# stm233/image-compression-for-machine

Hardware: AMD Instinct MI355X
Metric: images/sec (256x256) cnn-hyperprior (WACNN) training step (higher is better)
Workload: dtype f32; 1 GPU; cnn (WACNN N=192 M=320) train step, lambda=0.0067 MSE, batch 16/GPU synthetic 256x256, Adam lr 1e-4 + aux Adam, clip 1.0; global_batch=16, parallelism=dp1

## Files before the change

image-compression-for-machine_amd/csrc/conv_1x1.hip:

```cpp
#include <cstdlib>
#include "conv_common.h"

namespace icm {

template <int TCO, int TPX>
__global__ __launch_bounds__(256, 2) void conv1x1_kernel(const ConvDesc d) {
  constexpr int DB = 4;
  const int lane = threadIdx.x & 63;
  const int wave = __builtin_amdgcn_readfirstlane((int)(threadIdx.x >> 6));
  const ConvPtrs P = d.g[blockIdx.y];
  int bid = xcd_block_id();
  const int cb = bid % d.ncb, ptile = bid / d.ncb;
  const int h = lane >> 5, l31 = lane & 31;
  const int HW = d.pg.H * d.pg.W;
  const int NP = d.pg.N * HW;
  const int p_base = (ptile * 4 + wave) * (32 * TPX);
  if (p_base >= NP) return;
  unsigned voff[TPX];
  int pn[TPX], phw[TPX];
  bool pv[TPX];
#pragma unroll
  for (int tp = 0; tp < TPX; ++tp) {
    const int p = p_base + tp * 32 + l31;
    pv[tp] = p < NP;
// ... 44 lines not shown
      const int q = q0 + u;
      if (q >= nq) break;
      float bv[4][TPX];
#pragma unroll
      for (int j = 0; j < 4; ++j)
#pragma unroll
        for (int tp = 0; tp < TPX; ++tp) bv[j][tp] = bq[u][j][tp];
      if (act == ICM_ACT_GELU) {
#pragma unroll
        for (int j = 0; j < 4; ++j)
#pragma unroll
          for (int tp = 0; tp < TPX; ++tp) bv[j][tp] = gelu_f(bv[j][tp]);
      } else if (act == ICM_ACT_SQUARE) {
#pragma unroll
        for (int j = 0; j < 4; ++j)
#pragma unroll
          for (int tp = 0; tp < TPX; ++tp) bv[j][tp] *= bv[j][tp];
      }
      loadB(bq[u], q + DB);
      const char* sp = wbase + (long long)min(q + 2, nq - 1) * qstride;
#pragma unroll
      for (int a = 0; a < TCO; ++a) {
#pragma unroll
        for (int tp = 0; tp < TPX; ++tp)
#pragma unroll
          for (int j = 0; j < 4; ++j)
            acc[a][tp] = __builtin_amdgcn_mfma_f32_32x32x2f32(aq[u & 1][a][j], bv[j][tp], acc[a][tp], 0, 0, 0);
        aq[u & 1][a] = *reinterpret_cast<const f32x4*>(sp + wl[a]);
        __builtin_amdgcn_sched_barrier(0);
      }
    }
  }

  int zero[TPX];
#pragma unroll
  for (int tp = 0; tp < TPX; ++tp) zero[tp] = 0;
  epilogue_dispatch<TCO, TPX, !(TCO == 3 && TPX == 2)>(d, P, acc, cot0, h, pn, zero, phw, pv);
}

struct Cfg1x1 {
  int tco, tpx;
  void (*fn)(const ConvDesc);
  float eff;
};
static const Cfg1x1 kCfgs1x1[] = {
    {6, 1, conv1x1_kernel<6, 1>, 1.0f},  {5, 1, conv1x1_kernel<5, 1>, 1.0f}, {4, 1, conv1x1_kernel<4, 1>, 0.97f},
    {3, 2, conv1x1_kernel<3, 2>, 1.0f},  {2, 2, conv1x1_kernel<2, 2>, 0.7f}, {1, 2, conv1x1_kernel<1, 2>, 0.6f},
    {3, 1, conv1x1_kernel<3, 1>, 0.95f}, {2, 1, conv1x1_kernel<2, 1>, 0.6f},
};

int plan_conv1x1(const icm_conv_args& a, int ngroups, int g_force_1x1, ConvPlan& p) {
  if (g_force_1x1 == 0) return -1;
  if (a.KH != 1 || a.KW != 1 || a.stride != 1 || a.pad != 0 || a.pixel_shuffle || (a.Cin % 8) != 0) return -1;
  if (a.OH != a.H || a.OW != a.W) return -1;
  const int ncot = cdiv(a.Cout, 32);
  const long long NP = (long long)a.N * a.H * a.W;
  int best = -1, best_pad = 1 << 30;
  const int ncfg = (int)(sizeof(kCfgs1x1) / sizeof(kCfgs1x1[0]));
  for (int i = 0; i < ncfg; ++i) best_pad = std::min(best_pad, cdiv(ncot, kCfgs1x1[i].tco) * kCfgs1x1[i].tco);
  float best_score = -1.0f;
  for (int i = 0; i < ncfg; ++i) {
    const Cfg1x1& k = kCfgs1x1[i];
    if (cdiv(ncot, k.tco) * k.tco != best_pad) continue;
    const long long waves = ((NP + 32 * k.tpx - 1) / (32 * k.tpx)) * cdiv(ncot, k.tco) * ngroups;
    const float score = (float)std::min<long long>(waves, 2048) * k.eff;
    if (score > best_score) {
      best_score = score;
      best = i;
    }
  }
  {
    static const int force = env_int("ICM_1X1_CFG", -1);
    if (force >= 0 && force < ncfg) best = force;
  }
  const Cfg1x1& c = kCfgs1x1[best];
  const int ncb = cdiv(ncot, c.tco);
  const long long strips = (NP + 32 * c.tpx - 1) / (32 * c.tpx);
  static const long long kMinWaves = env_ll("ICM_1X1_MIN_WAVES", 1024);
  static const int kShortK = env_int("ICM_1X1_SHORT_K", 384);
  const long long need = a.Cin <= kShortK ? kMinWaves / 2 : kMinWaves;
  if (g_force_1x1 < 0 && strips * ncb * ngroups < need) return -1;
  const long long nblk = ((strips + 3) / 4) * ncb;
  if (nblk <= 0 || nblk > 0x7fffffffLL) return ICM_ERR_ARG;
  p = ConvPlan{};
  p.family = kFam1x1; p.row = best; p.g.ckm = 1; p.ncb = ncb; p.nblk = nblk; p.block = 256;
  return ICM_OK;
}

int launch_conv1x1(ConvDesc& d, const icm_conv_args& a, const ConvPlan& p, int ngroups, hipStream_t stream) {
  d.pg.H = a.H; d.pg.W = a.W; d.pg.N = a.N; d.pg.C = a.Cin; d.pg.act = a.pro_act; d.pg.bs = a.x_bs;
  d.OHf = a.H; d.OWf = a.W; d.OHv = a.H; d.OWv = a.W;
  d.out_sy = d.out_sx = 1;
  d.ntaps = 1;
  d.tiles_x = d.tiles_y = d.tiles_n = 1;
  d.nchunks8 = a.Cin / 8; d.ckm = p.g.ckm;
  hipLaunchKernelGGL(kCfgs1x1[p.row].fn, dim3((unsigned)p.nblk, ngroups, 1), dim3(p.block), 0, stream, d);
  ICM_CHECK_LAUNCH();
  return ICM_OK;
}

}
```

image-compression-for-machine_amd/csrc/conv_common.h:

```cpp
#pragma once
#include <type_traits>
#include "icm_common.h"

namespace icm {

#define ICM_MAX_TAPS 32
#define ICM_MAX_GROUPS 12

struct ConvPtrs {
  const float* x;
  const float* wp;
  const float* bias;
  float* y;
  const float* res;
  const float* aux;
  const float* aux2;
  float* y2;
};

struct ConvDesc {
  ConvPtrs g[ICM_MAX_GROUPS];
  long long y_bs, res_bs, aux_bs, aux2_bs, y2_bs;
  PatchGeom pg;
  int Cout, OHf, OWf;
  int OHv, OWv;
  int out_sy, out_oy, out_sx, out_ox;
  int iy0, ix0;
  int ntaps;
  int lgTW, lgTH, lgTI;
  int tiles_x, tiles_y, tiles_n;
  int ncot, nchunks8, ckm, ncb;
  int epi, accum, ps2;
  int tapoff[ICM_MAX_TAPS];
};

inline void fill_conv_ptrs(ConvPtrs (&g)[ICM_MAX_GROUPS], const icm_conv_args* arr, int ngroups, long long wp_off) {
  for (int gi = 0; gi < ICM_MAX_GROUPS; ++gi) {
    const icm_conv_args& s = arr[gi < ngroups ? gi : 0];
    g[gi] = ConvPtrs{s.x, s.wp + wp_off, s.bias, s.y, s.res, s.aux, s.aux2, s.y2};
  }
}
inline void fill_conv_desc(ConvDesc& d, const icm_conv_args* arr, int ngroups, long long wp_off) {
  const icm_conv_args& a = arr[0];
  fill_conv_ptrs(d.g, arr, ngroups, wp_off);
  d.y_bs = a.y_bs; d.res_bs = a.res_bs; d.aux_bs = a.aux_bs; d.aux2_bs = a.aux2_bs; d.y2_bs = a.y2_bs;
  d.Cout = a.Cout; d.ncot = (a.Cout + 31) / 32;
  d.epi = a.epi; d.accum = a.accum;
}

enum ConvFamily { kFamStaged = 0, kFamKs8 = 1, kFam1x1 = 2, kFamWino44 = 3, kFamWino8 = 4 };
struct Geometry {
  int lgTW, lgTH, lgTI, PH, PW, PWh, PWrow, PP, CS, tiles_x, tiles_y, tiles_n, ckm;
  size_t lds_bytes;
};
struct ConvPlan {
  int family;
  int row;
  Geometry g;
  int ncb;
  long long nblk;
  int block, vec4, dma;
};
struct WinoGeom {
  int lgTX, lgTY, lgTI, tiles_x, tiles_y, tiles_n, nchunks8, nsteps;
};
struct WinoPlan {
  WinoGeom g;
  int tco, w8, px_fast, ncb;
  long long nblk;
  size_t lds_bytes;
};

constexpr bool epi_reads_res(int e) { return e == ICM_EPI_RES || e == ICM_EPI_RES_GELU || e == ICM_EPI_RES_MUL_DGELU; }
constexpr bool epi_reads_aux(int e) {
  return e == ICM_EPI_GDN || e == ICM_EPI_IGDN || e == ICM_EPI_MUL_DGELU || e == ICM_EPI_AXPY2 || e == ICM_EPI_LRP ||
         e == ICM_EPI_RES_MUL_DGELU;
}
constexpr bool epi_reads_aux2(int e) { return e == ICM_EPI_AXPY2; }
constexpr bool epi_writes_side(int e) { return e == ICM_EPI_GDN || e == ICM_EPI_IGDN || e == ICM_EPI_LRP; }
constexpr bool epi_may_gelu(int e) { return e == ICM_EPI_NONE || e == ICM_EPI_RES || e == ICM_EPI_RES_GELU; }

template <int EPI>
__device__ __forceinline__ float epi_apply(float v, float rv, float av, float& side) {
  if constexpr (EPI == ICM_EPI_RES) v += rv;
  if constexpr (EPI == ICM_EPI_RES_GELU) v += gelu_f(rv);
  if constexpr (EPI == ICM_EPI_GDN || EPI == ICM_EPI_IGDN) {
    side = v;
    v = av * (EPI == ICM_EPI_GDN ? rsqrtf(v) : sqrtf(v));
  }
  if constexpr (EPI == ICM_EPI_MUL_DGELU) v *= dgelu_f(av);
  if constexpr (EPI == ICM_EPI_RES_MUL_DGELU) v = (v + rv) * dgelu_f(av);
  if constexpr (EPI == ICM_EPI_AXPY2) v = rv + 2.0f * av * v;
  if constexpr (EPI == ICM_EPI_LRP) {
    side = tanhf(v);
    v = av + 0.5f * side;
  }
  return v;
}
template <class Off>
__device__ __forceinline__ void epi_materialise(float& v, const float* y, float* y2, Off off, bool ok) {
  const float gv = gelu_f(v);
  if (y2 == y) v = gv;
  else if (ok) y2[off] = gv;
}

template <int... Kinds>
struct EpiKinds {
  static constexpr bool has(int epi) { return ((epi == Kinds) || ...); }
  template <class F>
  static __device__ __forceinline__ void dispatch(int epi, F&& f) {
    static_assert(((Kinds == ICM_EPI_NONE) || ...), "ICM_EPI_NONE is the fallback of every kernel");
    const bool hit = ((Kinds != ICM_EPI_NONE && epi == Kinds ? (f(std::integral_constant<int, Kinds>{}), true) : false) || ...);
    if (!hit) f(std::integral_constant<int, ICM_EPI_NONE>{});
  }
};
using EpiAll = EpiKinds<ICM_EPI_NONE, ICM_EPI_RES, ICM_EPI_RES_GELU, ICM_EPI_GDN, ICM_EPI_IGDN, ICM_EPI_MUL_DGELU,
                        ICM_EPI_AXPY2, ICM_EPI_LRP, ICM_EPI_RES_MUL_DGELU>;
using EpiKs8 = EpiKinds<ICM_EPI_NONE, ICM_EPI_RES, ICM_EPI_RES_GELU, ICM_EPI_MUL_DGELU, ICM_EPI_LRP, ICM_EPI_RES_MUL_DGELU>;
using EpiWino = EpiKinds<ICM_EPI_NONE, ICM_EPI_RES, ICM_EPI_RES_GELU, ICM_EPI_MUL_DGELU, ICM_EPI_RES_MUL_DGELU, ICM_EPI_LRP>;

template <int EPI, int half>
__device__ __forceinline__ void store_half_e(const ConvDesc& d, const ConvPtrs& P, const f32x16 acc, int cot, int h,
                                             int n, int oy, int ox, bool pvalid) {
  const int plane = d.OHf * d.OWf;
  constexpr bool kRes = epi_reads_res(EPI), kAux = epi_reads_aux(EPI), kAux2 = epi_reads_aux2(EPI);
  float* yb = P.y + n * d.y_bs;
  const float* resb = kRes ? P.res + n * d.res_bs : nullptr;
  const float* auxb = kAux ? P.aux + n * d.aux_bs : nullptr;
  const float* aux2b = kAux2 ? P.aux2 + n * d.aux2_bs : nullptr;
  float* y2b = P.y2 ? P.y2 + n * d.y2_bs : nullptr;
  const bool has_bias = P.bias != nullptr;
  {
    int off[8];
    bool ok[8];
    float bv[8], rv[8], av[8];
#pragma unroll
// ... 120 lines not shown
      }
    return;
  }
  constexpr int S = TPX * TCO * 2;
  EpiRegs R[2];
  epi_load<EPI>(d, P, cot0, 0, h, pn[0], poy[0], pox[0], pv[0], R[0]);
#pragma unroll
  for (int i = 0; i < S; ++i) {
    const int half = i & 1, a = (i >> 1) % TCO, tp = (i >> 1) / TCO;
    if (i + 1 < S) {
      const int i2 = i + 1;
      const int half2 = i2 & 1, a2 = (i2 >> 1) % TCO, tp2 = (i2 >> 1) / TCO;
      epi_load<EPI>(d, P, cot0 + a2, half2, h, pn[tp2], poy[tp2], pox[tp2], pv[tp2], R[i2 & 1]);
    }
    __builtin_amdgcn_sched_barrier(0);
    float a8[8];
#pragma unroll
    for (int q = 0; q < 8; ++q) a8[q] = acc[a][tp][half * 8 + q];
    epi_finish<EPI>(d, P, a8, R[i & 1]);
    __builtin_amdgcn_sched_barrier(0);
  }
}

template <int TCO, int TPX, bool PIPE2 = false>
__device__ __forceinline__ void epilogue_dispatch(const ConvDesc& d, const ConvPtrs& P, const f32x16 (&acc)[TCO][TPX],
                                                  int cot0, int h, const int (&pn)[TPX], const int (&poy)[TPX],
                                                  const int (&pox)[TPX], const bool (&pv)[TPX]) {
  EpiAll::dispatch(d.epi, [&](auto kind) {
    constexpr int EPI = decltype(kind)::value;
    epilogue_tiles<EPI, TCO, TPX, EPI == ICM_EPI_AXPY2 && PIPE2>(d, P, acc, cot0, h, pn, poy, pox, pv);
  });
}

int launch_conv_ks8(const ConvDesc& d, int tco, long long nblk, int ngroups, size_t lds_bytes, hipStream_t stream);

bool wino_supported(const icm_conv_args& a);
int plan_conv_wino(const icm_conv_args& a, int ngroups, WinoPlan& p);
int run_conv_wino(const icm_conv_args* arr, int ngroups, hipStream_t stream);
long long wino_transform_floats(const icm_conv_args& a);
int run_wino_transform(const icm_conv_args* arr, int ngroups, hipStream_t stream);

int plan_conv1x1(const icm_conv_args& a, int ngroups, int force_mode, ConvPlan& p);
int launch_conv1x1(ConvDesc& d, const icm_conv_args& a, const ConvPlan& p, int ngroups, hipStream_t stream);

}
```

image-compression-for-machine_amd/csrc/conv_igemm.hip:

```cpp
#include <climits>
#include <cstdlib>
#include <vector>
#include "conv_common.h"

namespace icm {

template <int WCO, int WPX, int TCO, int TPX, int KS = 1>
__global__ __launch_bounds__(512, (TCO * TPX <= 3) ? 4 : 2) void conv_igemm_kernel(const ConvDesc d) {
  extern __shared__ __attribute__((aligned(16))) float smem[];
  static_assert(WCO * WPX * KS == 4, "4 MFMA waves per workgroup");
  constexpr int BCO_T = WCO * TCO;
  constexpr int TS = (TCO * TPX == 1) ? 3 : ((TCO * TPX == 2) ? 2 : 1);
  const int tid = threadIdx.x, lane = tid & 63, wave = tid >> 6;
  const bool loader = wave >= 4;
  const ConvPtrs P = d.g[blockIdx.y];
  const PatchGeom& pg = d.pg;

  int bid = xcd_block_id();
  const int cb = bid % d.ncb;
  int pt = bid / d.ncb;
  const int tx_i = pt % d.tiles_x;
  pt /= d.tiles_x;
  const int ty_i = pt % d.tiles_y;
  const int tn_i = pt / d.tiles_y;
// ... 464 lines not shown
    }
    if (cost < best_cost) {
      best_cost = cost;
      best = i;
      bg = g;
    }
  }
  if (best1 >= 0 && best1_cost <= 1.2 * best_cost) {
    best = best1;
    bg = bg1;
  }
  return best;
}

static int plan_ks8(const icm_conv_args& a, int ngroups, const ConvClass& cls, const ClassShape& s, int S_in, Geometry& g) {
  static const int ks8_on = env_int("ICM_CONV_KS8", 1);
  static const long long ks8_max = env_ll("ICM_CONV_KS8_MAXWG", 256);
  static const long long ks8_min = env_ll("ICM_CONV_KS8_MINWG", 160);
  if (!(ks8_forced() || (ks8_on && !cfg_forced())) || S_in != 1 || s.ntaps <= 1 || a.pro_act != ICM_ACT_NONE ||
      !EpiKs8::has(a.epi) || a.x_seg_len != 0)
    return 0;
  const int tco = g_force_cfg == ICM_CONV_CFG_KS8_32X128 ? 1 : (g_force_cfg == ICM_CONV_CFG_KS8_64X64 ? 2 : (s.ncot >= 2 ? 2 : 1));
  g = make_geometry(tco == 2 ? 64 : 128, s.OHv, s.OWv, a.N, S_in, cls.ey, cls.ex, s.nchunks8, s.ntaps, 4);
  int ckm = std::max(1, std::min(s.nchunks8, 64 / s.ntaps));
  while (ckm > 1 && (size_t)2 * ckm * 8 * g.CS * sizeof(float) > 96 * 1024) --ckm;
  g.ckm = ckm;
  g.lds_bytes = std::max((size_t)2 * ckm * 8 * g.CS * sizeof(float), (size_t)8 * 4 * 16 * 64 * sizeof(float));
  const long long blocks = cdiv(s.ncot, tco) * tile_count(g) * ngroups;
  const bool fits = g.lds_bytes <= 160 * 1024 && fits_plane_map(g) && linear_patch(g);
  return (fits && (ks8_forced() || (blocks <= ks8_max && blocks >= ks8_min && tco == 2))) ? tco : 0;
}

static int plan_class(const icm_conv_args& a, int ngroups, const ConvClass& cls, int S_in, int out_s, bool x_aligned16,
                      ConvPlan& p) {
  p = ConvPlan{};
  const ClassShape s = class_shape(a, cls, out_s);
  if (s.OHv <= 0 || s.OWv <= 0) return ICM_OK;
  if (s.ntaps > ICM_MAX_TAPS) return ICM_ERR_UNSUPPORTED;
  if (s.ntaps == 1 && S_in == 1 && out_s == 1 && cls.iy0 == 0 && cls.ix0 == 0 && a.x_seg_len == 0 && !cfg_forced()) {
    const int rc = plan_conv1x1(a, ngroups, g_force_1x1, p);
    if (rc >= 0) return rc;
  }
  p.row = search_staged(a, ngroups, cls, s, S_in, p.g);
  if (p.row < 0) return ICM_ERR_UNSUPPORTED;
  p.block = 512;
  Geometry kg;
  if (const int tco = plan_ks8(a, ngroups, cls, s, S_in, kg)) {
    p.family = kFamKs8;
    p.row = tco;
    p.g = kg;
    p.dma = 1;
  } else {
    const Geometry& g = p.g;
    const int plane4 = (1 << g.lgTI) * g.PH * (g.PW / 4);
    p.vec4 = S_in == 1 && cls.ex == 1 && cls.ey == 1 && cls.ix0 == 0 && (g.PW % 4) == 0 && ((1 << g.lgTW) % 4) == 0 &&
             (a.W % 4) == 0 && (a.x_bs % 4) == 0 && ((long long)a.H * a.W % 4) == 0 && plane4 <= 4 * 64 &&
             (g.CS % 4) == 0 && (g.PWrow % 4) == 0 && (g.PP % 4) == 0 && x_aligned16 && a.x_seg_len == 0;
    static const int dma_on = env_int("ICM_CONV_DMA", 1);
    p.dma = dma_on && !p.vec4 && S_in == 1 && a.pro_act == ICM_ACT_NONE && linear_patch(g);
  }
  p.ncb = cdiv(s.ncot, p.family == kFamKs8 ? p.row : kCfgs[p.row].wco * kCfgs[p.row].tco);
  p.nblk = p.ncb * tile_count(p.g);
  if (p.nblk <= 0 || p.nblk > 0x7fffffffLL) return ICM_ERR_ARG;
  return ICM_OK;
}

static int launch_class(const icm_conv_args* arr, int ngroups, const ConvClass& cls, long long wp_off, int S_in,
                        int out_s, const ConvPlan& p, hipStream_t stream) {
  if (p.nblk == 0) return ICM_OK;
  const icm_conv_args& a = arr[0];
  ConvDesc d{};
  fill_conv_desc(d, arr, ngroups, wp_off);
  d.ncb = p.ncb;
// ... 61 lines not shown
  }
  const icm_conv_args& a = arr[0];
  for (int i = 1; i < ngroups; ++i) {
    const icm_conv_args& b = arr[i];
    if (b.N != a.N || b.Cin != a.Cin || b.H != a.H || b.W != a.W || b.Cout != a.Cout || b.OH != a.OH || b.OW != a.OW ||
        b.KH != a.KH || b.KW != a.KW || b.stride != a.stride || b.pad != a.pad || b.transposed != a.transposed ||
        b.pro_act != a.pro_act || b.epi != a.epi || b.accum != a.accum || b.pixel_shuffle != a.pixel_shuffle ||
        b.x_bs != a.x_bs || b.y_bs != a.y_bs || b.x_seg_len != a.x_seg_len || b.x_seg_gap != a.x_seg_gap || b.algo != a.algo ||
        (b.res && b.res_bs != a.res_bs) || (b.aux && b.aux_bs != a.aux_bs) || (b.aux2 && b.aux2_bs != a.aux2_bs) ||
        (b.y2 && b.y2_bs != a.y2_bs) || (b.res != nullptr) != (a.res != nullptr) || (b.aux != nullptr) != (a.aux != nullptr) ||
        (b.aux2 != nullptr) != (a.aux2 != nullptr) || (b.y2 != nullptr) != (a.y2 != nullptr) ||
        (b.bias != nullptr) != (a.bias != nullptr) || (b.xv != nullptr) != (a.xv != nullptr))
      return ICM_ERR_ARG;
  }
  return (a.algo == ICM_ALGO_WINOGRAD || a.algo == ICM_ALGO_DIRECT) ? ICM_OK : ICM_ERR_ARG;
}

static long long class_packed_floats(int Cin, int ntaps, int ncot) { return (long long)cdiv(Cin, 8) * ntaps * ncot * 256; }

static bool x_aligned16(const icm_conv_args* arr, int ngroups) {
  bool ok = true;
  for (int gi = 0; gi < ngroups; ++gi) ok = ok && (reinterpret_cast<uintptr_t>(arr[gi].x) & 15) == 0;
  return ok;
}

static int conv_run_grouped(const icm_conv_args* arr, int ngroups, hipStream_t stream) {
  if (int rc = check_group(arr, ngroups)) return rc;
  const icm_conv_args& a = arr[0];
  if (a.algo == ICM_ALGO_WINOGRAD) return run_conv_wino(arr, ngroups, stream);
  const int S_in = a.transposed ? 1 : a.stride, out_s = a.transposed ? a.stride : 1;
  long long off = 0;
  for (const ConvClass& cls : build_classes(a.KH, a.KW, a.stride, a.pad, a.transposed)) {
    ConvPlan p;
    int rc = plan_class(a, ngroups, cls, S_in, out_s, x_aligned16(arr, ngroups), p);
    if (!rc) rc = launch_class(arr, ngroups, cls, off, S_in, out_s, p, stream);
    if (rc) return rc;
    off += class_packed_floats(a.Cin, (int)cls.taps.size(), cdiv(a.Cout, 32));
  }
  return ICM_OK;
}

static PackDesc make_pack_desc(const icm_pack_job& J, const ConvClass& cls, long long off) {
  const int ntaps = (int)cls.taps.size(), ncot = cdiv(J.Cout, 32);
  PackDesc d{};
  d.w = J.w;
  d.wp = J.wp + off;
  d.Co = J.Cout; d.Ci = J.Cin; d.KHW = J.KH * J.KW; d.src_out_major = J.src_out_major;
  d.ntaps = ntaps; d.ncot = ncot; d.nchunks = cdiv(J.Cin, 8); d.nonneg = J.nonneg;
  d.bound = J.bound; d.pedestal = J.pedestal;
  d.src_ld = J.src_ld > 0 ? J.src_ld : (J.src_out_major ? J.Cin : J.Cout); d.src_off = J.src_off;
  d.dst_ncot = J.dst_ncot > 0 ? J.dst_ncot : ncot; d.dst_cot_off = J.dst_cot_off; d.wino = J.wino;
  d.cg = d.KHW == 1 ? 4 : 1;
  d.ngroups = cdiv(d.nchunks, d.cg);
  d.vec = (reinterpret_cast<uintptr_t>(J.w) & 15) == 0 && ((long long)d.src_ld * d.KHW) % 4 == 0 &&
          ((long long)d.src_off * d.KHW) % 4 == 0;
  for (int t = 0; t < ntaps; ++t) d.tapidx[t] = (short)cls.taps[t].kidx;
  return d;
}
static int pack_items(const PackDesc& d) { return d.ncot * d.ngroups; }
static size_t pack_lds_bytes(const PackDesc& d) { return sizeof(float) * pack_lds_floats(d.cg, d.KHW); }

}

extern "C" {

int icm_conv_run(const icm_conv_args* a, void* stream) {
  return icm::conv_run_grouped(a, 1, (hipStream_t)stream);
// ... 26 lines not shown
  if (!arr || ngroups < 1 || ngroups > ICM_MAX_GROUPS) return ICM_ERR_ARG;
  for (int i = 1; i < ngroups; ++i)
    if (arr[i].N != arr[0].N || arr[i].Cin != arr[0].Cin || arr[i].H != arr[0].H || arr[i].W != arr[0].W ||
        arr[i].x_bs != arr[0].x_bs || arr[i].pro_act != arr[0].pro_act || arr[i].x_seg_len != arr[0].x_seg_len ||
        arr[i].x_seg_gap != arr[0].x_seg_gap)
      return ICM_ERR_ARG;
  return icm::run_wino_transform(arr, ngroups, (hipStream_t)stream);
}

void icm_debug_force_conv_cfg(int idx) { icm::g_force_cfg = idx < 0 ? ICM_CONV_CFG_AUTO : idx; }
int icm_debug_forced_conv_cfg(void) { return icm::g_force_cfg; }
void icm_debug_force_conv1x1(int mode) { icm::g_force_1x1 = mode; }

int icm_debug_conv_plan(const icm_conv_args* arr, int ngroups, int cls, int64_t out[16]) {
  using namespace icm;
  std::fill(out, out + 16, 0);
  int rc = check_group(arr, ngroups);
  if (rc) return rc;
  const icm_conv_args& a = arr[0];
  if (a.algo == ICM_ALGO_WINOGRAD) {
    WinoPlan w{};
    if (cls != 0) return ICM_ERR_ARG;
    if ((rc = plan_conv_wino(a, ngroups, w))) return rc;
    const int64_t v[13] = {1, w.w8 ? kFamWino8 : kFamWino44, w.tco, w.g.lgTX, w.g.lgTY, w.g.lgTI, w.g.nsteps, w.ncb, w.nblk,
                           (int64_t)w.lds_bytes, 512, a.xv != nullptr, w.px_fast};
    std::copy(v, v + 13, out);
    return ICM_OK;
  }
  const std::vector<ConvClass> classes = build_classes(a.KH, a.KW, a.stride, a.pad, a.transposed);
  if (cls < 0 || cls >= (int)classes.size()) return ICM_ERR_ARG;
  long long off = 0;
  for (int i = 0; i < cls; ++i) off += class_packed_floats(a.Cin, (int)classes[i].taps.size(), cdiv(a.Cout, 32));
  ConvPlan p;
  rc = plan_class(a, ngroups, classes[cls], a.transposed ? 1 : a.stride, a.transposed ? a.stride : 1, x_aligned16(arr, ngroups), p);
  if (rc) return rc;
  const int64_t v[14] = {(int64_t)classes.size(), p.family, p.row, p.g.lgTW, p.g.lgTH, p.g.lgTI, p.g.ckm, p.ncb, p.nblk,
                         (int64_t)p.g.lds_bytes, p.block, p.vec4, p.dma, off};
  std::copy(v, v + 14, out);
  return ICM_OK;
}

int64_t icm_packed_weight_floats(int Cout, int Cin, int KH, int KW) {
  return icm::class_packed_floats(Cin, KH * KW, icm::cdiv(Cout, 32));
}

int icm_pack_weights(const float* w, float* wp, int Cout, int Cin, int KH, int KW, int src_out_major,
                     int transposed, int stride, int pad, int nonneg, float bound, float pedestal, void* stream) {
  using namespace icm;
  if (!w || !wp || Cout <= 0 || Cin <= 0 || KH * KW > ICM_MAX_TAPS || (stride != 1 && stride != 2)) return ICM_ERR_ARG;
  icm_pack_job J{};
  J.w = w; J.wp = wp; J.Cout = Cout; J.Cin = Cin; J.KH = KH; J.KW = KW; J.src_out_major = src_out_major; J.nonneg = nonneg;
  J.bound = bound; J.pedestal = pedestal;
  long long off = 0;
  for (const ConvClass& cls : build_classes(KH, KW, stride, pad, transposed)) {
    if (cls.taps.empty()) continue;
    const PackDesc d = make_pack_desc(J, cls, off);
    hipLaunchKernelGGL(pack_weights_kernel, dim3(pack_items(d)), dim3(256), pack_lds_bytes(d), (hipStream_t)stream, d);
    ICM_CHECK_LAUNCH();
    off += class_packed_floats(Cin, d.ntaps, d.dst_ncot);
  }
  return ICM_OK;
}

int icm_pack_weights_batch(const icm_pack_job* jobs, int n, void* stream) {
  using namespace icm;
  if (!jobs || n < 1) return ICM_ERR_ARG;
  PackMulti m{};
  int nb = 0;
  auto flush = [&]() -> int {
    if (nb == 0) return ICM_OK;
    long long items = 0;
    size_t lds = 0;
// ... 45 lines not shown
```

image-compression-for-machine_amd/icm_amd/_lib.py:

```python
from __future__ import annotations

import ctypes as C
import os

import torch

_HERE = os.path.dirname(os.path.abspath(__file__))
LIB_PATH = os.environ.get("ICM_LIB", os.path.join(os.path.dirname(_HERE), "lib", "libicm_hip.so"))

ACT_NONE, ACT_GELU, ACT_SQUARE = 0, 1, 2
CONV_CFG_AUTO, CONV_CFG_KS8_64X64, CONV_CFG_KS8_32X128 = -1, 100, 101
TILE_EDGE_LEFT, TILE_EDGE_RIGHT, TILE_EDGE_TOP, TILE_EDGE_BOTTOM = 1, 2, 4, 8
EPI_NONE, EPI_RES, EPI_RES_GELU, EPI_GDN, EPI_IGDN, EPI_MUL_DGELU, EPI_AXPY2, EPI_LRP, EPI_RES_MUL_DGELU = range(9)

_f = C.POINTER(C.c_float)
i64, i32, f32, vp = C.c_int64, C.c_int, C.c_float, C.c_void_p


class ConvArgs(C.Structure):
    _fields_ = [
        ("x", vp), ("x_bs", i64), ("N", i32), ("Cin", i32), ("H", i32), ("W", i32),
        ("wp", vp), ("bias", vp),
        ("y", vp), ("y_bs", i64), ("Cout", i32), ("OH", i32), ("OW", i32),
        ("KH", i32), ("KW", i32), ("stride", i32), ("pad", i32),
# ... 14 lines not shown
    ]


class PackJob(C.Structure):
    _fields_ = [("w", vp), ("wp", vp), ("Cout", i32), ("Cin", i32), ("KH", i32), ("KW", i32), ("src_out_major", i32),
                ("transposed", i32), ("stride", i32), ("pad", i32), ("nonneg", i32), ("bound", f32), ("pedestal", f32),
                ("src_ld", i32), ("src_off", i32), ("dst_ncot", i32), ("dst_cot_off", i32), ("wino", i32)]


class EbParams(C.Structure):
    _fields_ = [("matrix", vp * 5), ("bias", vp * 5), ("factor", vp * 4), ("quantiles", vp)]


class EbGrads(C.Structure):
    _fields_ = [("matrix", vp * 5), ("bias", vp * 5), ("factor", vp * 4), ("dmedian", vp)]


class IcmError(RuntimeError):
    pass


_lib = None

SYMBOLS = [
    "icm_strerror", "icm_version", "icm_conv_run", "icm_conv_run_grouped", "icm_conv2d_fwd", "icm_conv2d_dgrad",
    "icm_convT2d_fwd", "icm_convT2d_dgrad", "icm_packed_weight_floats", "icm_pack_weights", "icm_pack_weights_batch",
    "icm_wgrad_workspace_floats", "icm_wgrad_workspace_floats_grouped", "icm_conv_wgrad", "icm_conv_wgrad_grouped", "icm_channel_sum", "icm_nonneg_fwd", "icm_nonneg_bwd",
    "icm_gdn_bwd_pre", "icm_gelu_fwd", "icm_gate_fwd", "icm_gate_bwd", "icm_add_grad", "icm_ste_round_offset",
    "icm_lrp_bwd", "icm_pixel_unshuffle2", "icm_layernorm_fwd", "icm_layernorm_bwd", "icm_space_to_depth2",
    "icm_residual_scale", "icm_im2col", "icm_col2im", "icm_copy_strided", "icm_permute_flip", "icm_gather_vectors", "icm_conv_winograd_ok", "icm_wino_transform_floats", "icm_wino_transform", "icm_winattn_fwd", "icm_winattn_bwd",
    "icm_eb_likelihood_fwd", "icm_eb_likelihood_bwd", "icm_eb_aux_loss", "icm_gc_likelihood_ste_fwd",
    "icm_gc_likelihood_ste_bwd", "icm_rd_loss_fwd", "icm_rd_loss_bwd", "icm_grad_sqnorm", "icm_adam_step", "icm_adam_step_hyper", "icm_fill",
    "icm_winattn_bwd_workspace_floats", "icm_debug_force_conv_cfg", "icm_debug_forced_conv_cfg", "icm_debug_force_conv1x1",
    "icm_debug_force_wgrad_cfg", "icm_debug_wgrad_plan", "icm_debug_conv_plan",
    "icm_debug_force_winattn_valu", "icm_debug_winattn_route",
    "icm_zigzag_order", "icm_zigzag_splits", "icm_zigzag_reverse",
    "icm_pmf_to_quantized_cdf", "icm_rans_encode_with_indexes", "icm_rans_decode_with_indexes",
    "icm_rans_decoder_create", "icm_rans_decoder_decode", "icm_rans_decoder_destroy",
    "icm_rans_lanes_waves", "icm_rans_lanes_encode", "icm_rans_lanes_decoder_create",
    "icm_rans_lanes_decoder_decode_run", "icm_rans_lanes_decoder_finish", "icm_rans_lanes_decoder_destroy",
    "icm_rans_lanes_encode_gpu_workspace", "icm_rans_lanes_encode_gpu", "icm_rans_lanes_decoder_gpu_create",
    "icm_rans_lanes_decoder_gpu_decode_run", "icm_rans_lanes_decoder_gpu_finish", "icm_rans_lanes_decoder_gpu_destroy",
    "icm_debug_lanes_search",
    "icm_eb_table_bounds", "icm_eb_pmf_table", "icm_gc_table_centers", "icm_gc_pmf_table", "icm_gc_build_indexes",
    "icm_quantize", "icm_dequantize", "icm_clamp", "icm_pad2d",
    "icm_gc_code_q", "icm_gc_indexes_q", "icm_dequantize_q",
    "icm_gc_code_qmap", "icm_gc_indexes_qmap", "icm_dequantize_qmap", "icm_gc_code_rdo",
    "icm_gc_likelihood_ste_qs_fwd", "icm_gc_likelihood_ste_qs_bwd", "icm_rd_loss_w_fwd", "icm_rd_loss_w_bwd",
    "icm_gc_likelihood_ste_qm_fwd", "icm_gc_likelihood_ste_qm_bwd", "icm_rd_loss_m_fwd", "icm_rd_loss_m_bwd",
    "icm_qmap_paint",
    "icm_msssim_workspace_floats", "icm_msssim_fwd", "icm_msssim_bwd",
    "icm_image_workspace_bytes", "icm_image_u8_to_f32", "icm_image_f32_to_u8",
    "icm_image_batch_u8_to_f32", "icm_image_tile_blend",
]
REDUCE_WS_FLOATS = 8192


def lib():
    global _lib
    if _lib is None:
        if not os.path.exists(LIB_PATH):
            raise IcmError(
                f"{LIB_PATH} not found: build it with image-compression-for-machine_amd/build.sh "
                "(hipcc --offload-arch=gfx950). There is no CPU fallback.")
        L = C.CDLL(LIB_PATH)
        L.icm_strerror.restype = C.c_char_p
        L.icm_packed_weight_floats.restype = i64
# ... 14 lines not shown
        L.icm_wgrad_workspace_floats_grouped.argtypes = [C.POINTER(WgradArgs), i32]
        L.icm_conv_wgrad.argtypes = [C.POINTER(WgradArgs), vp]
        L.icm_conv_wgrad_grouped.argtypes = [C.POINTER(WgradArgs), i32, vp]
        L.icm_channel_sum.argtypes = [vp, i64, i32, i32, i32, vp, i32, vp, i64, vp]
        L.icm_gather_vectors.argtypes = [C.POINTER(vp), i32, i32, vp, vp]
        L.icm_nonneg_fwd.argtypes = [vp, vp, i64, f32, f32, vp]
        L.icm_nonneg_bwd.argtypes = [vp, vp, vp, i64, f32, i32, vp]
        L.icm_gdn_bwd_pre.argtypes = [vp, vp, vp, vp, vp, i64, i32, vp]
        L.icm_gelu_fwd.argtypes = [vp, vp, i64, vp]
        L.icm_gate_fwd.argtypes = [vp, vp, vp, vp, i64, vp]
        L.icm_gate_bwd.argtypes = [vp, vp, vp, vp, vp, vp, i64, i32, i32, vp]
        L.icm_add_grad.argtypes = [vp, vp, vp, i64, i32, vp]
        L.icm_ste_round_offset.argtypes = [vp, vp, vp, i32, i32, i32, vp]
        L.icm_lrp_bwd.argtypes = [vp, i64, vp, i64, vp, i64, i32, i32, i32, vp]
        L.icm_pixel_unshuffle2.argtypes = [vp, vp, i32, i32, i32, i32, vp]
        L.icm_layernorm_fwd.argtypes = [vp, i64, vp, vp, vp, i64, vp, vp, i32, i32, i32, f32, vp]
        L.icm_layernorm_bwd.argtypes = [vp, i64, vp, i64, vp, vp, vp, vp, i64, vp, vp, i32, i32, i32, i32, i32, vp, i64,
                                        vp, i64, vp]
        L.icm_space_to_depth2.argtypes = [vp, vp, i32, i32, i32, i32, i32, i32, vp]
        L.icm_residual_scale.argtypes = [vp, vp, vp, vp, i32, i64, vp]
        L.icm_im2col.argtypes = [vp, vp, i32, i32, i32, i32, i32, i32, i32, vp]
        L.icm_col2im.argtypes = [vp, vp, vp, i32, i32, i32, i32, i32, i32, i32, i32, vp]
        L.icm_copy_strided.argtypes = [vp, i64, vp, i64, i32, i32, i32, i32, vp]
        L.icm_permute_flip.argtypes = [vp, vp, i32, i32, i32, i32, vp]
        L.icm_winattn_fwd.argtypes = [vp, vp, vp, i32, i32, i32, i32, i32, i32, i32, vp]
        L.icm_winattn_bwd.argtypes = [vp, vp, vp, vp, vp, i32, vp, i64, i32, i32, i32, i32, i32, i32, i32, vp]
        L.icm_winattn_bwd_workspace_floats.argtypes = [i32, i32, i32, i32, i32, i32]
        L.icm_winattn_bwd_workspace_floats.restype = i64
        L.icm_debug_force_conv_cfg.argtypes = [i32]
        L.icm_debug_force_conv_cfg.restype = None
        L.icm_debug_force_conv1x1.argtypes = [i32]
        L.icm_debug_force_conv1x1.restype = None
        L.icm_debug_conv_plan.argtypes = [C.POINTER(ConvArgs), i32, i32, C.POINTER(i64)]
        L.icm_debug_force_wgrad_cfg.argtypes = [i32, i32]
        L.icm_debug_force_wgrad_cfg.restype = None
        L.icm_debug_wgrad_plan.argtypes = [C.POINTER(WgradArgs), i32, C.POINTER(C.c_int32)]
        L.icm_debug_force_winattn_valu.argtypes = [i32]
        L.icm_debug_force_winattn_valu.restype = None
        L.icm_debug_winattn_route.argtypes = [i32, i32, i32, i32, i32, i32, i32, i32]
        L.icm_eb_likelihood_fwd.argtypes = [vp, vp, C.POINTER(EbParams), vp, vp, i32, i32, i32, f32, vp]
        L.icm_eb_likelihood_bwd.argtypes = [vp, vp, C.POINTER(EbParams), vp, vp, C.POINTER(EbGrads), i32, i32, i32,
                                            f32, i32, vp]
        L.icm_eb_aux_loss.argtypes = [C.POINTER(EbParams), vp, vp, i32, f32, vp]
        L.icm_gc_likelihood_ste_fwd.argtypes = [vp, i64, vp, i64, vp, i64, vp, i64, vp, i64, vp, i64, vp, i64, i32,
                                                i32, i32, f32, f32, vp]
        L.icm_gc_likelihood_ste_bwd.argtypes = [vp, i64, vp, i64, vp, i64, vp, i64, vp, i64, vp, i64, vp, i64, vp,
                                                i64, vp, i64, i32, i32, i32, f32, f32, i32, vp]
        L.icm_rd_loss_fwd.argtypes = [vp, vp, i64, vp, i64, vp, i64, i64, f32, vp, vp, vp]
        L.icm_rd_loss_bwd.argtypes = [vp, vp, i64, vp, i64, vp, i64, i64, f32, f32, vp, vp, vp, vp]
        L.icm_gc_likelihood_ste_qs_fwd.argtypes = [vp, i64, vp, i64, vp, i64, vp, i64, vp, vp, i64, vp, i64, vp, i64, i32,
                                                   i32, i32, f32, f32, vp]
        L.icm_gc_likelihood_ste_qs_bwd.argtypes = [vp, i64, vp, i64, vp, i64, vp, i64, vp, vp, i64, vp, i64, vp, i64, vp,
                                                   i64, vp, i64, i32, i32, i32, f32, f32, i32, vp]
        L.icm_rd_loss_w_fwd.argtypes = [vp, vp, i32, i64, vp, i64, vp, i64, i64, vp, vp, vp, vp]
        L.icm_rd_loss_w_bwd.argtypes = [vp, vp, i32, i64, vp, i64, vp, i64, i64, vp, f32, vp, vp, vp, vp]
        L.icm_gc_likelihood_ste_qm_fwd.argtypes = [vp, i64, vp, i64, vp, i64, vp, i64, vp, vp, vp, i64, vp, i64, vp, i64,
                                                   i32, i32, i32, f32, f32, vp]
        L.icm_gc_likelihood_ste_qm_bwd.argtypes = [vp, i64, vp, i64, vp, i64, vp, i64, vp, vp, vp, i64, vp, i64, vp, i64,
                                                   vp, i64, vp, i64, i32, i32, i32, f32, f32, i32, vp]
        L.icm_rd_loss_m_fwd.argtypes = [vp, vp, i32, i32, i32, i32, i32, vp, vp, vp, i64, vp, i64, i64, vp, vp, vp]
        L.icm_rd_loss_m_bwd.argtypes = [vp, vp, i32, i32, i32, i32, i32, vp, vp, vp, i64, vp, i64, i64, f32, vp, vp, vp,
                                        vp]
        L.icm_qmap_paint.argtypes = [vp, vp, i32, vp, i32, i32, i32, vp]
        L.icm_grad_sqnorm.argtypes = [vp, i64, vp, vp, vp]
        L.icm_adam_step.argtypes = [vp, vp, vp, vp, i64, C.c_double, C.c_double, C.c_double, C.c_double, i32, vp, f32, f32, vp]
        L.icm_adam_step_hyper.argtypes = [vp, vp, vp, vp, i64, C.c_double, C.c_double, C.c_double, vp, vp, f32, f32, vp]
# ... 96 lines not shown
```

include/icm_hip.h:

```cpp
#ifndef ICM_HIP_H
#define ICM_HIP_H
#include <stdint.h>

#ifdef __cplusplus
extern "C" {
#endif

#define ICM_OK 0
#define ICM_ERR_ARG 1
#define ICM_ERR_LAUNCH 2
#define ICM_ERR_UNSUPPORTED 3

#define ICM_ACT_NONE 0
#define ICM_ACT_GELU 1
#define ICM_ACT_SQUARE 2

#define ICM_EPI_NONE 0
#define ICM_EPI_RES 1
#define ICM_EPI_RES_GELU 2
#define ICM_EPI_GDN 3
#define ICM_EPI_IGDN 4
#define ICM_EPI_MUL_DGELU 5
#define ICM_EPI_AXPY2 6
#define ICM_EPI_LRP 7
// ... 268 lines not shown
int icm_adam_step(float* p, const float* g, float* m, float* v, int64_t n, double lr, double beta1, double beta2,
                  double eps, int step, const float* sqnorm, float max_norm, float gscale, void* stream);
int icm_adam_step_hyper(float* p, const float* g, float* m, float* v, int64_t n, double beta1, double beta2, double eps,
                        const float* hyper, const float* sqnorm, float max_norm, float gscale, void* stream);
int icm_fill(float* p, int64_t n, float v, void* stream);
int icm_clamp(float* p, int64_t n, float lo, float hi, void* stream);
int icm_pad2d(const float* src, int N, int C, int H, int W, float* dst, int OH, int OW, int top, int left, float value,
              void* stream);

int64_t icm_image_workspace_bytes(int H, int W);
int icm_image_u8_to_f32(const uint8_t* src, int H, int W, float* dst, int OH, int OW, int top, int left, void* stream);
int icm_image_f32_to_u8(const float* src, int PH, int PW, int top, int left, uint8_t* dst, int H, int W,
                        const uint8_t* ref, int64_t* sse, void* ws, int64_t ws_bytes, void* stream);

#define ICM_TILE_EDGE_LEFT 1
#define ICM_TILE_EDGE_RIGHT 2
#define ICM_TILE_EDGE_TOP 4
#define ICM_TILE_EDGE_BOTTOM 8
int icm_image_tile_blend(const float* src, int PH, int PW, int top, int left, int h, int w,
                         float* canvas, int H, int W, int y0, int x0,
                         const float* ramp, int m, int edges, void* stream);

typedef struct { int64_t offset; int32_t H, W, y0, x0; } icm_crop_desc;
int icm_image_batch_u8_to_f32(const uint8_t* arena, const icm_crop_desc* desc, int B, float* dst ,
                              int CH, int CW, void* stream);

#define ICM_CONV_CFG_AUTO (-1)
#define ICM_CONV_CFG_KS8_64X64 100
#define ICM_CONV_CFG_KS8_32X128 101
void icm_debug_force_conv_cfg(int idx);
int icm_debug_forced_conv_cfg(void);
void icm_debug_force_conv1x1(int mode);
int icm_debug_conv_plan(const icm_conv_args* a, int ngroups, int cls, int64_t out[16]);
void icm_debug_force_wgrad_cfg(int variant, int xcd_order);
int icm_debug_wgrad_plan(const icm_wgrad_args* a, int n, int32_t out[8]);
void icm_debug_force_winattn_valu(int on);
int icm_debug_winattn_route(int N, int C, int H, int W, int heads, int ws, int shift, int backward);

#ifdef __cplusplus
}
#endif
#endif
```

Before: 406.3 images/s.

## Add vectorised wide epilogue for 1x1 conv using quad DPP transpose

Adds a wide epilogue path for the 1x1 MFMA conv kernel. It transposes accumulator fragments across lane quads with DPP so each lane holds four consecutive pixels, then does 16-byte loads and stores for outputs, residual, aux and accumulate operands in place of scalar accesses. A double-buffered prefetch of the epilogue operands overlaps with the transpose, and pinned dgelu/unfused-add helpers try to keep rounding identical to the scalar path. It is enabled when pointers and strides are 16-byte aligned and H*W is a multiple of 4, at the cost of extra registers and code complexity.

```diff
diff --git a/image-compression-for-machine_amd/csrc/conv_1x1.hip b/image-compression-for-machine_amd/csrc/conv_1x1.hip
--- a/image-compression-for-machine_amd/csrc/conv_1x1.hip
+++ b/image-compression-for-machine_amd/csrc/conv_1x1.hip
@@ -100,6 +100,19 @@
     }
   }
 
+  if (d.wide) {
+    int qn[TPX], qhw[TPX];
+    bool qv[TPX];
+#pragma unroll
+    for (int tp = 0; tp < TPX; ++tp) {
+      qv[tp] = p_base + tp * 32 + (l31 & ~3) < NP;
+      qn[tp] = pn[tp];
+      qhw[tp] = phw[tp] - (l31 & 3);
+    }
+    constexpr int kPcs = TCO * TPX >= 6 ? 2 : 4;
+    epilogue_dispatch_wide<TCO, TPX, kPcs>(d, P, acc, cot0, h, l31 & 3, qn, qhw, qv);
+    return;
+  }
   int zero[TPX];
 #pragma unroll
   for (int tp = 0; tp < TPX; ++tp) zero[tp] = 0;
@@ -155,6 +168,22 @@
   return ICM_OK;
 }
 
+bool conv1x1_wide_ok(const icm_conv_args* arr, int ngroups) {
+  const icm_conv_args& a = arr[0];
+  if (((long long)a.H * a.W) % 4 != 0) return false;
+  auto al = [](const void* p, long long bs) { return (reinterpret_cast<uintptr_t>(p) & 15) == 0 && bs % 4 == 0; };
+  const bool uses_y2 = epi_writes_side(a.epi) || epi_may_gelu(a.epi);
+  for (int gi = 0; gi < ngroups; ++gi) {
+    const icm_conv_args& s = arr[gi];
+    if (!al(s.y, s.y_bs)) return false;
+    if (epi_reads_res(a.epi) && !al(s.res, s.res_bs)) return false;
+    if (epi_reads_aux(a.epi) && !al(s.aux, s.aux_bs)) return false;
+    if (epi_reads_aux2(a.epi) && !al(s.aux2, s.aux2_bs)) return false;
+    if (uses_y2 && s.y2 && !al(s.y2, s.y2_bs)) return false;
+  }
+  return true;
+}
+
 int launch_conv1x1(ConvDesc& d, const icm_conv_args& a, const ConvPlan& p, int ngroups, hipStream_t stream) {
   d.pg.H = a.H; d.pg.W = a.W; d.pg.N = a.N; d.pg.C = a.Cin; d.pg.act = a.pro_act; d.pg.bs = a.x_bs;
   d.OHf = a.H; d.OWf = a.W; d.OHv = a.H; d.OWv = a.W;
@@ -162,6 +191,7 @@
   d.ntaps = 1;
   d.tiles_x = d.tiles_y = d.tiles_n = 1;
   d.nchunks8 = a.Cin / 8; d.ckm = p.g.ckm;
+  d.wide = p.wide;
   hipLaunchKernelGGL(kCfgs1x1[p.row].fn, dim3((unsigned)p.nblk, ngroups, 1), dim3(p.block), 0, stream, d);
   ICM_CHECK_LAUNCH();
   return ICM_OK;
diff --git a/image-compression-for-machine_amd/csrc/conv_common.h b/image-compression-for-machine_amd/csrc/conv_common.h
--- a/image-compression-for-machine_amd/csrc/conv_common.h
+++ b/image-compression-for-machine_amd/csrc/conv_common.h
@@ -31,6 +31,7 @@
   int tiles_x, tiles_y, tiles_n;
   int ncot, nchunks8, ckm, ncb;
   int epi, accum, ps2;
+  int wide;
   int tapoff[ICM_MAX_TAPS];
 };
 
@@ -60,6 +61,7 @@
   int ncb;
   long long nblk;
   int block, vec4, dma;
+  int wide;
 };
 struct WinoGeom {
   int lgTX, lgTY, lgTI, tiles_x, tiles_y, tiles_n, nchunks8, nsteps;
@@ -80,16 +82,32 @@
 constexpr bool epi_writes_side(int e) { return e == ICM_EPI_GDN || e == ICM_EPI_IGDN || e == ICM_EPI_LRP; }
 constexpr bool epi_may_gelu(int e) { return e == ICM_EPI_NONE || e == ICM_EPI_RES || e == ICM_EPI_RES_GELU; }
 
-template <int EPI>
-__device__ __forceinline__ float epi_apply(float v, float rv, float av, float& side) {
+struct DgeluAsWritten {
+  __device__ __forceinline__ float operator()(float x) const { return dgelu_f(x); }
+};
+__device__ __forceinline__ float dgelu_two_roundings(float x, float pdf, float cdf) {
+#pragma clang fp contract(off)
+  return cdf + x * pdf;
+}
+struct DgeluPinned {
+  bool two_roundings;
+  __device__ __forceinline__ float operator()(float x) const {
+    const float cdf = 0.5f * (1.0f + erf_bf(x * 0.70710678118654752440f));
+    const float pdf = 0.39894228040143267794f * __builtin_amdgcn_exp2f(-0.72134752044448170f * x * x);
+    return two_roundings ? dgelu_two_roundings(x, pdf, cdf) : fmaf(x, pdf, cdf);
+  }
+};
+
+template <int EPI, class Dgelu = DgeluAsWritten>
+__device__ __forceinline__ float epi_apply(float v, float rv, float av, float& side, Dgelu dgelu = Dgelu{}) {
   if constexpr (EPI == ICM_EPI_RES) v += rv;
   if constexpr (EPI == ICM_EPI_RES_GELU) v += gelu_f(rv);
   if constexpr (EPI == ICM_EPI_GDN || EPI == ICM_EPI_IGDN) {
     side = v;
     v = av * (EPI == ICM_EPI_GDN ? rsqrtf(v) : sqrtf(v));
   }
-  if constexpr (EPI == ICM_EPI_MUL_DGELU) v *= dgelu_f(av);
-  if constexpr (EPI == ICM_EPI_RES_MUL_DGELU) v = (v + rv) * dgelu_f(av);
+  if constexpr (EPI == ICM_EPI_MUL_DGELU) v *= dgelu(av);
+  if constexpr (EPI == ICM_EPI_RES_MUL_DGELU) v = (v + rv) * dgelu(av);
   if constexpr (EPI == ICM_EPI_AXPY2) v = rv + 2.0f * av * v;
   if constexpr (EPI == ICM_EPI_LRP) {
     side = tanhf(v);
@@ -97,11 +115,15 @@
   }
   return v;
 }
+__device__ __forceinline__ float epi_materialise_value(float& v, bool same) {
+  const float gv = gelu_f(v);
+  if (same) v = gv;
+  return gv;
+}
 template <class Off>
 __device__ __forceinline__ void epi_materialise(float& v, const float* y, float* y2, Off off, bool ok) {
-  const float gv = gelu_f(v);
-  if (y2 == y) v = gv;
-  else if (ok) y2[off] = gv;
+  const float gv = epi_materialise_value(v, y2 == y);
+  if (y2 != y && ok) y2[off] = gv;
 }
 
 template <int... Kinds>
@@ -288,6 +310,158 @@
   });
 }
 
+
+template <int CTRL>
+__device__ __forceinline__ float quad_perm_f(float v) {
+  const int i = __builtin_bit_cast(int, v);
+  return __builtin_bit_cast(float, __builtin_amdgcn_update_dpp(i, i, CTRL, 0xf, 0xf, false));
+}
+__device__ __forceinline__ void quad_transpose4(float (&a)[4], int j) {
+  const bool o1 = (j & 1) != 0, o2 = (j & 2) != 0;
+#pragma unroll
+  for (int p = 0; p < 4; p += 2) {
+    const float r = quad_perm_f<0xB1>(o1 ? a[p] : a[p + 1]);
+    a[p] = o1 ? r : a[p];
+    a[p + 1] = o1 ? a[p + 1] : r;
+  }
+#pragma unroll
+  for (int p = 0; p < 2; ++p) {
+    const float r = quad_perm_f<0x4E>(o2 ? a[p] : a[p + 2]);
+    a[p] = o2 ? r : a[p];
+    a[p + 2] = o2 ? a[p + 2] : r;
+  }
+}
+
+__device__ __forceinline__ float add_unfused(float a, float b) {
+#pragma clang fp contract(off)
+  return a + b;
+}
+
+template <int PCS>
+struct WideRegs {
+  int n;
+  int off[PCS];
+  bool ok[PCS];
+  bool dg2[PCS];
+  float bv[PCS];
+  f32x4 rv[PCS], av[PCS], old[PCS];
+};
+
+template <int EPI, int PCS>
+__device__ __forceinline__ void wide_load(const ConvDesc& d, const ConvPtrs& P, int cot, int m0, int h, int j, int n, int hw,
+                                          bool pvalid, WideRegs<PCS>& R) {
+  const int plane = d.OHf * d.OWf;
+  constexpr bool kRes = epi_reads_res(EPI), kAux = epi_reads_aux(EPI), kAux2 = epi_reads_aux2(EPI);
+  const float* yb = P.y + n * d.y_bs;
+  const float* resb = kRes ? P.res + n * d.res_bs : nullptr;
+  const float* auxb = kAux ? P.aux + n * d.aux_bs : nullptr;
+  const float* aux2b = kAux2 ? P.aux2 + n * d.aux2_bs : nullptr;
+  const bool has_bias = P.bias != nullptr;
+  const bool tile_ok = pvalid && cot < d.ncot;
+  const f32x4 z = {0.0f, 0.0f, 0.0f, 0.0f};
+  R.n = n;
+#pragma unroll
+  for (int q = 0; q < PCS; ++q) {
+    const int co = cot * 32 + j + 8 * (m0 + q) + 4 * h;
+    R.ok[q] = tile_ok && co < d.Cout;
+    R.dg2[q] = j == 3 && ((m0 + q) & 1) != 0;
+    R.off[q] = co * plane + hw;
+    R.bv[q] = (has_bias && R.ok[q]) ? P.bias[co] : 0.0f;
+    if constexpr (kRes) R.rv[q] = R.ok[q] ? *reinterpret_cast<const f32x4*>(resb + R.off[q]) : z;
+    if constexpr (kAux) R.av[q] = R.ok[q] ? *reinterpret_cast<const f32x4*>(auxb + R.off[q]) : z;
+    if constexpr (kAux2) R.rv[q] = R.ok[q] ? *reinterpret_cast<const f32x4*>(aux2b + R.off[q]) : z;
+  }
+  if (d.accum) {
+#pragma unroll
+    for (int q = 0; q < PCS; ++q) R.old[q] = R.ok[q] ? *reinterpret_cast<const f32x4*>(yb + R.off[q]) : z;
+  }
+}
+
+template <int EPI, int PCS>
+__device__ __forceinline__ void wide_finish(const ConvDesc& d, const ConvPtrs& P, const float (&t)[PCS][4],
+                                            const WideRegs<PCS>& R) {
+  float* yb = P.y + R.n * d.y_bs;
+  float* y2b = P.y2 ? P.y2 + R.n * d.y2_bs : nullptr;
+  constexpr bool kRv = epi_reads_res(EPI) || epi_reads_aux2(EPI), kAux = epi_reads_aux(EPI);
+  f32x4 v[PCS];
+#pragma unroll
+  for (int q = 0; q < PCS; ++q) {
+    f32x4 side;
+#pragma unroll
+    for (int e = 0; e < 4; ++e) {
+      float s;
+      v[q][e] = epi_apply<EPI>(t[q][e] + R.bv[q], kRv ? R.rv[q][e] : 0.0f, kAux ? R.av[q][e] : 0.0f, s,
+                               DgeluPinned{EPI == ICM_EPI_MUL_DGELU && R.dg2[q]});
+      if constexpr (epi_writes_side(EPI)) side[e] = s;
+    }
+    if constexpr (epi_writes_side(EPI))
+      if (y2b && R.ok[q]) *reinterpret_cast<f32x4*>(y2b + R.off[q]) = side;
+  }
+  if (d.accum) {
+#pragma unroll
+    for (int q = 0; q < PCS; ++q)
+#pragma unroll
+      for (int e = 0; e < 4; ++e) v[q][e] = add_unfused(v[q][e], R.old[q][e]);
+  }
+  if constexpr (epi_may_gelu(EPI)) {
+    if (y2b) {
+      const bool same = y2b == yb;
+#pragma unroll
+      for (int q = 0; q < PCS; ++q) {
+        f32x4 gv;
+#pragma unroll
+        for (int e = 0; e < 4; ++e) {
+          float ve = v[q][e];
+          gv[e] = epi_materialise_value(ve, same);
+          v[q][e] = ve;
+        }
+        if (!same && R.ok[q]) *reinterpret_cast<f32x4*>(y2b + R.off[q]) = gv;
+      }
+    }
+  }
+#pragma unroll
+  for (int q = 0; q < PCS; ++q)
+    if (R.ok[q]) *reinterpret_cast<f32x4*>(yb + R.off[q]) = v[q];
+}
+
+template <int EPI, int TCO, int TPX, int PCS>
+__device__ __forceinline__ void epilogue_tiles_wide(const ConvDesc& d, const ConvPtrs& P, const f32x16 (&acc)[TCO][TPX],
+                                                    int cot0, int h, int j, const int (&qn)[TPX], const int (&qhw)[TPX],
+                                                    const bool (&qv)[TPX]) {
+  constexpr int SPT = 4 / PCS, S = TPX * TCO * SPT;
+  WideRegs<PCS> R[2];
+  wide_load<EPI, PCS>(d, P, cot0, 0, h, j, qn[0], qhw[0], qv[0], R[0]);
+#pragma unroll
+  for (int i = 0; i < S; ++i) {
+    const int m0 = (i % SPT) * PCS, a = (i / SPT) % TCO, tp = (i / SPT) / TCO;
+    if (i + 1 < S) {
+      const int i2 = i + 1;
+      const int m2 = (i2 % SPT) * PCS, a2 = (i2 / SPT) % TCO, tp2 = (i2 / SPT) / TCO;
+      wide_load<EPI, PCS>(d, P, cot0 + a2, m2, h, j, qn[tp2], qhw[tp2], qv[tp2], R[i2 & 1]);
+    }
+    __builtin_amdgcn_sched_barrier(0);
+    float t[PCS][4];
+#pragma unroll
+    for (int q = 0; q < PCS; ++q) {
+#pragma unroll
+      for (int e = 0; e < 4; ++e) t[q][e] = acc[a][tp][4 * (m0 + q) + e];
+      quad_transpose4(t[q], j);
+    }
+    wide_finish<EPI, PCS>(d, P, t, R[i & 1]);
+    __builtin_amdgcn_sched_barrier(0);
+  }
+}
+
+template <int TCO, int TPX, int PCS>
+__device__ __forceinline__ void epilogue_dispatch_wide(const ConvDesc& d, const ConvPtrs& P, const f32x16 (&acc)[TCO][TPX],
+                                                       int cot0, int h, int j, const int (&qn)[TPX], const int (&qhw)[TPX],
+                                                       const bool (&qv)[TPX]) {
+  EpiAll::dispatch(d.epi, [&](auto kind) {
+    constexpr int EPI = decltype(kind)::value;
+    epilogue_tiles_wide<EPI, TCO, TPX, PCS>(d, P, acc, cot0, h, j, qn, qhw, qv);
+  });
+}
+
 int launch_conv_ks8(const ConvDesc& d, int tco, long long nblk, int ngroups, size_t lds_bytes, hipStream_t stream);
 
 bool wino_supported(const icm_conv_args& a);
@@ -297,6 +471,7 @@
 int run_wino_transform(const icm_conv_args* arr, int ngroups, hipStream_t stream);
 
 int plan_conv1x1(const icm_conv_args& a, int ngroups, int force_mode, ConvPlan& p);
+bool conv1x1_wide_ok(const icm_conv_args* arr, int ngroups);
 int launch_conv1x1(ConvDesc& d, const icm_conv_args& a, const ConvPlan& p, int ngroups, hipStream_t stream);
 
 }
diff --git a/image-compression-for-machine_amd/csrc/conv_igemm.hip b/image-compression-for-machine_amd/csrc/conv_igemm.hip
--- a/image-compression-for-machine_amd/csrc/conv_igemm.hip
+++ b/image-compression-for-machine_amd/csrc/conv_igemm.hip
@@ -520,13 +520,14 @@
 }
 
 static int plan_class(const icm_conv_args& a, int ngroups, const ConvClass& cls, int S_in, int out_s, bool x_aligned16,
-                      ConvPlan& p) {
+                      bool wide_ok, ConvPlan& p) {
   p = ConvPlan{};
   const ClassShape s = class_shape(a, cls, out_s);
   if (s.OHv <= 0 || s.OWv <= 0) return ICM_OK;
   if (s.ntaps > ICM_MAX_TAPS) return ICM_ERR_UNSUPPORTED;
   if (s.ntaps == 1 && S_in == 1 && out_s == 1 && cls.iy0 == 0 && cls.ix0 == 0 && a.x_seg_len == 0 && !cfg_forced()) {
     const int rc = plan_conv1x1(a, ngroups, g_force_1x1, p);
+    if (rc == ICM_OK) p.wide = wide_ok;
     if (rc >= 0) return rc;
   }
   p.row = search_staged(a, ngroups, cls, s, S_in, p.g);
@@ -654,7 +655,7 @@
   long long off = 0;
   for (const ConvClass& cls : build_classes(a.KH, a.KW, a.stride, a.pad, a.transposed)) {
     ConvPlan p;
-    int rc = plan_class(a, ngroups, cls, S_in, out_s, x_aligned16(arr, ngroups), p);
+    int rc = plan_class(a, ngroups, cls, S_in, out_s, x_aligned16(arr, ngroups), conv1x1_wide_ok(arr, ngroups), p);
     if (!rc) rc = launch_class(arr, ngroups, cls, off, S_in, out_s, p, stream);
     if (rc) return rc;
     off += class_packed_floats(a.Cin, (int)cls.taps.size(), cdiv(a.Cout, 32));
@@ -747,12 +748,24 @@
   long long off = 0;
   for (int i = 0; i < cls; ++i) off += class_packed_floats(a.Cin, (int)classes[i].taps.size(), cdiv(a.Cout, 32));
   ConvPlan p;
-  rc = plan_class(a, ngroups, classes[cls], a.transposed ? 1 : a.stride, a.transposed ? a.stride : 1, x_aligned16(arr, ngroups), p);
+  rc = plan_class(a, ngroups, classes[cls], a.transposed ? 1 : a.stride, a.transposed ? a.stride : 1, x_aligned16(arr, ngroups),
+                  conv1x1_wide_ok(arr, ngroups), p);
   if (rc) return rc;
   const int64_t v[14] = {(int64_t)classes.size(), p.family, p.row, p.g.lgTW, p.g.lgTH, p.g.lgTI, p.g.ckm, p.ncb, p.nblk,
                          (int64_t)p.g.lds_bytes, p.block, p.vec4, p.dma, off};
   std::copy(v, v + 14, out);
   return ICM_OK;
+}
+
+int icm_debug_conv1x1_wide(const icm_conv_args* arr, int ngroups) {
+  using namespace icm;
+  if (check_group(arr, ngroups) || arr[0].algo == ICM_ALGO_WINOGRAD) return 0;
+  const icm_conv_args& a = arr[0];
+  const std::vector<ConvClass> classes = build_classes(a.KH, a.KW, a.stride, a.pad, a.transposed);
+  ConvPlan p;
+  const int rc = plan_class(a, ngroups, classes[0], a.transposed ? 1 : a.stride, a.transposed ? a.stride : 1,
+                            x_aligned16(arr, ngroups), conv1x1_wide_ok(arr, ngroups), p);
+  return rc == ICM_OK && p.nblk > 0 && p.family == kFam1x1 && p.wide;
 }
 
 int64_t icm_packed_weight_floats(int Cout, int Cin, int KH, int KW) {
diff --git a/image-compression-for-machine_amd/icm_amd/_lib.py b/image-compression-for-machine_amd/icm_amd/_lib.py
--- a/image-compression-for-machine_amd/icm_amd/_lib.py
+++ b/image-compression-for-machine_amd/icm_amd/_lib.py
@@ -70,7 +70,7 @@
     "icm_eb_likelihood_fwd", "icm_eb_likelihood_bwd", "icm_eb_aux_loss", "icm_gc_likelihood_ste_fwd",
     "icm_gc_likelihood_ste_bwd", "icm_rd_loss_fwd", "icm_rd_loss_bwd", "icm_grad_sqnorm", "icm_adam_step", "icm_adam_step_hyper", "icm_fill",
     "icm_winattn_bwd_workspace_floats", "icm_debug_force_conv_cfg", "icm_debug_forced_conv_cfg", "icm_debug_force_conv1x1",
-    "icm_debug_force_wgrad_cfg", "icm_debug_wgrad_plan", "icm_debug_conv_plan",
+    "icm_debug_force_wgrad_cfg", "icm_debug_wgrad_plan", "icm_debug_conv_plan", "icm_debug_conv1x1_wide",
     "icm_debug_force_winattn_valu", "icm_debug_winattn_route",
     "icm_zigzag_order", "icm_zigzag_splits", "icm_zigzag_reverse",
     "icm_pmf_to_quantized_cdf", "icm_rans_encode_with_indexes", "icm_rans_decode_with_indexes",
@@ -151,6 +151,8 @@
         L.icm_debug_force_conv1x1.argtypes = [i32]
         L.icm_debug_force_conv1x1.restype = None
         L.icm_debug_conv_plan.argtypes = [C.POINTER(ConvArgs), i32, i32, C.POINTER(i64)]
+        if hasattr(L, "icm_debug_conv1x1_wide"):
+            L.icm_debug_conv1x1_wide.argtypes = [C.POINTER(ConvArgs), i32]
         L.icm_debug_force_wgrad_cfg.argtypes = [i32, i32]
         L.icm_debug_force_wgrad_cfg.restype = None
         L.icm_debug_wgrad_plan.argtypes = [C.POINTER(WgradArgs), i32, C.POINTER(C.c_int32)]
diff --git a/include/icm_hip.h b/include/icm_hip.h
--- a/include/icm_hip.h
+++ b/include/icm_hip.h
@@ -324,6 +324,7 @@
 int icm_debug_forced_conv_cfg(void);
 void icm_debug_force_conv1x1(int mode);
 int icm_debug_conv_plan(const icm_conv_args* a, int ngroups, int cls, int64_t out[16]);
+int icm_debug_conv1x1_wide(const icm_conv_args* a, int ngroups);
 void icm_debug_force_wgrad_cfg(int variant, int xcd_order);
 int icm_debug_wgrad_plan(const icm_wgrad_args* a, int n, int32_t out[8]);
 void icm_debug_force_winattn_valu(int on);
```

Measured after the change: 416.5 images/s (median of 5 runs). 2.5% higher.
